# lucidrains/phenaki-pytorch

Measured on AMD Instinct MI355X. Metric: cvivit_encode_frames_per_sec, higher is better.
Workload: dtype bf16; 1 GPU; BASELINE configs[1]: C-ViViT (dim 512, patch 32, tpatch 2, depth 4+4, LFQ 65536) encode video -> token ids, (8,3,17,256,256) f32 per GPU resident in HBM; global_batch=8, parallelism=batch-shard x1, no data-path collective, hip_graph=True

## Files before the change

### phenaki_pytorch_amd/csrc/common.hpp

```cpp
#pragma once
#include <hip/hip_runtime.h>
#include <stdint.h>

namespace pk {

typedef float f32x4 __attribute__((ext_vector_type(4)));
typedef float f32x2 __attribute__((ext_vector_type(2)));
typedef __bf16 bf16x8_t __attribute__((ext_vector_type(8)));
typedef unsigned short u16;
typedef u16 u16x8 __attribute__((ext_vector_type(8)));
typedef u16 u16x4 __attribute__((ext_vector_type(4)));
typedef uint32_t u32x4 __attribute__((ext_vector_type(4)));
typedef uint32_t u32x2 __attribute__((ext_vector_type(2)));

struct bf16 { u16 v; };

struct bf16x3 { float v; };
struct bf16x3p { uint32_t v; };

typedef __bf16 bf16x2_native __attribute__((ext_vector_type(2)));
__device__ __forceinline__ u16 f2bf(float f) {
    return __builtin_bit_cast(u16, (__bf16)f);
}
__device__ __forceinline__ float bf2f(u16 h) {
// ... 104 lines not shown
}
__device__ __forceinline__ void store_elem(bf16x3p* p, float v) {
    const uintptr_t a = reinterpret_cast<uintptr_t>(p);
    char* blk = reinterpret_cast<char*>(a & ~(uintptr_t)127);
    const int o = (int)(a & 127) >> 1;
    const u16 h = f2bf(v);
    *reinterpret_cast<u16*>(blk + o) = h;
    *reinterpret_cast<u16*>(blk + 64 + o) = f2bf(v - bf2f(h));
}
__device__ __forceinline__ void store4(float* p, f32x4 v) { *reinterpret_cast<f32x4*>(p) = v; }
__device__ __forceinline__ void store4(bf16* p, f32x4 v) {
    *reinterpret_cast<u32x2*>(p) = u32x2{pack_bf2(v[0], v[1]), pack_bf2(v[2], v[3])};
}
__device__ __forceinline__ void store2(float* p, float a, float b) { *reinterpret_cast<f32x2*>(p) = f32x2{a, b}; }
__device__ __forceinline__ void store2(bf16* p, float a, float b) { *reinterpret_cast<uint32_t*>(p) = pack_bf2(a, b); }

__device__ __forceinline__ long xcd_contiguous_block(unsigned b, unsigned nblocks_padded) {
    return (long)(b & 7u) * (nblocks_padded >> 3) + (b >> 3);
}
__host__ __device__ inline unsigned xcd_padded_grid(long nblocks) { return (unsigned)(8 * ((nblocks + 7) / 8)); }

__device__ __forceinline__ float mul_rn(float a, float b) {
#pragma clang fp contract(off)
    return a * b;
}
__device__ __forceinline__ float add_rn(float a, float b) {
#pragma clang fp contract(off)
    return a + b;
}
__device__ __forceinline__ float wave_sum(float v) {
// ... 114 lines not shown
```

### phenaki_pytorch_amd/csrc/gemm.hip

```cpp
#include "gemm_dma.hpp"
#include "gemm_p8.hpp"

namespace pk {

enum { ACT_NONE = 0, ACT_GEGLU = 1, ACT_LEAKY = 2, ACT_RELU = 3 };

struct GemmEpilogue {
    const float* bias;
    const float* res;
    void* C;
    int ldr, ldc;
    int out_f32;
    int act;
    int vec_ok;
    void* C2;
    int ldc2;
    const float* ln_s; const float* ln_t; float ln_eps;
    const int* row_off; const int* col_off;
    float* stats_out; const float* ln_stats; int stats_np;
    int dup_rows;
};

constexpr int STATS_CHUNK = 32;

template <typename T, int TM, int TN, int WN>
__device__ __forceinline__ void gemm_epilogue_scalar(const f32x4 (&acc)[TM][TN], int M, int N, const GemmEpilogue& e, int m0, int n0) {
    const int lane = threadIdx.x & 63, wave = threadIdx.x >> 6;
    const int wm = wave / WN, wn = wave % WN, g = lane >> 4, lr = lane & 15;
    float* Cf = reinterpret_cast<float*>(e.C);
    T* Ct = reinterpret_cast<T*>(e.C);
#pragma unroll
    for (int i = 0; i < TM; ++i) {
        const int m = m0 + wm * 16 * TM + i * 16 + lr;
        if (m >= M) continue;
#pragma unroll
        for (int j = 0; j < TN; ++j) {
            const int n = n0 + wn * 16 * TN + j * 16 + g * 4;
            const f32x4 v = acc[i][j];
#pragma unroll
            for (int r = 0; r < 4; ++r) {
                const int nn = n + r;
                if (nn >= N) break;
                float x = v[r] + (e.bias ? e.bias[nn] : 0.f);
                if (e.act == ACT_GEGLU) {
                    if (r & 1) continue;
                    const float gate = (nn + 1 < N) ? v[r + 1] + (e.bias ? e.bias[nn + 1] : 0.f) : 0.f;
                    x = gelu_for<T>(gate) * x;
                    const size_t o = (size_t)m * e.ldc + (nn >> 1);
                    if (e.out_f32) Cf[o] = x; else store_elem(Ct + o, x);
                    continue;
                }
                if (e.act == ACT_LEAKY) x = x > 0.f ? x : 0.1f * x;
                if (e.act == ACT_RELU) x = fmaxf(x, 0.f);
                if (e.res) x += e.res[(size_t)m * e.ldr + nn];
                const size_t o = (size_t)m * e.ldc + nn;
                if (e.out_f32) Cf[o] = x; else store_elem(Ct + o, x);
            }
        }
    }
}

template <int TM> constexpr int epi_rows_per_round() { return TM > 2 ? 2 : TM; }

template <typename T, int TM, int TN, int WN = 2, bool LNF = false>
__device__ __forceinline__ void gemm_epilogue(const f32x4 (&acc)[TM][TN], int M, int N, const GemmEpilogue& e, int m0, int n0,
                                              const float* rsum = nullptr, const float* rsq = nullptr, int K = 1) {
    if (!e.vec_ok) {
        if (!LNF) gemm_epilogue_scalar<T, TM, TN, WN>(acc, M, N, e, m0, n0);
        return;
    }
    const int lane = threadIdx.x & 63, wave = threadIdx.x >> 6;
    const int wm = wave / WN, wn = wave % WN, g = lane >> 4, lr = lane & 15;
    float* __restrict__ Cf = reinterpret_cast<float*>(e.C);
    T* __restrict__ Ct = reinterpret_cast<T*>(e.C);
    const int mb = m0 + wm * 16 * TM + lr, nb = n0 + wn * 16 * TN + g * 4;
    f32x4 b4[TN], s4[TN], t4[TN];
    int coff[TN];
#pragma unroll
    for (int j = 0; j < TN; ++j) {
        const int nj = min(nb + j * 16, N - 4);
        b4[j] = e.bias ? *reinterpret_cast<const f32x4*>(e.bias + nj) : f32x4{0, 0, 0, 0};
        if (LNF) {
            s4[j] = *reinterpret_cast<const f32x4*>(e.ln_s + nj);
            t4[j] = *reinterpret_cast<const f32x4*>(e.ln_t + nj);
        }
        coff[j] = e.row_off ? e.col_off[nj] : nj;
    }
    constexpr int IB = epi_rows_per_round<TM>();
#pragma unroll
    for (int i0 = 0; i0 < TM; i0 += IB) {
        f32x4 r4[IB][TN];
        int roff[IB];
#pragma unroll
        for (int ii = 0; ii < IB; ++ii) {
            const int mi = min(mb + (i0 + ii) * 16, M - 1);
            roff[ii] = e.row_off ? e.row_off[mi] : 0;
            if (!LNF && e.res && e.act != ACT_GEGLU) {
#pragma unroll
                for (int j = 0; j < TN; ++j) r4[ii][j] = *reinterpret_cast<const f32x4*>(e.res + (size_t)mi * e.ldr + min(nb + j * 16, N - 4));
            } else {
#pragma unroll
                for (int j = 0; j < TN; ++j) r4[ii][j] = f32x4{0, 0, 0, 0};
            }
        }
#pragma unroll
        for (int ii = 0; ii < IB; ++ii) {
            const int i = i0 + ii, m = mb + i * 16;
            float mean = 0.f, rstd = 1.f;
            if (LNF) {
                const float inv_k = 1.0f / (float)K;
                mean = rsum[i] * inv_k;
                rstd = __builtin_amdgcn_rsqf(fmaxf(rsq[i] * inv_k - mean * mean, 0.f) + e.ln_eps);
            }
            float ps = 0.f, pq = 0.f;
#pragma unroll
            for (int j = 0; j < TN; ++j) {
                const int n = nb + j * 16;
                const bool live = m < M && n < N;
                f32x4 v = acc[i][j];
                if (LNF) {
#pragma unroll
                    for (int r = 0; r < 4; ++r) v[r] = rstd * (v[r] - mean * s4[j][r]) + t4[j][r];
                }
                v += b4[j];
                if (e.act == ACT_GEGLU) {
                    const float o0 = gelu_for<T>(v[1]) * v[0], o1 = gelu_for<T>(v[3]) * v[2];
                    const size_t o = (size_t)m * e.ldc + (n >> 1);
                    if (live) { if (e.out_f32) store2(Cf + o, o0, o1); else store2(Ct + o, o0, o1); }
                    continue;
                }
                if (e.act == ACT_LEAKY) {
#pragma unroll
                    for (int r = 0; r < 4; ++r) v[r] = v[r] > 0.f ? v[r] : 0.1f * v[r];
                }
                if (e.act == ACT_RELU) {
#pragma unroll
                    for (int r = 0; r < 4; ++r) v[r] = fmaxf(v[r], 0.f);
                }
                if (!LNF) v += r4[ii][j];
                else if (e.res && live) v += *reinterpret_cast<const f32x4*>(e.res + (size_t)m * e.ldr + n);
                if (live) {
                    const size_t o = e.row_off ? (size_t)((long)roff[ii] + (long)coff[j]) : (size_t)m * e.ldc + n;
                    if (e.out_f32) store4(Cf + o, v); else store4(Ct + o, v);
                    if (e.C2) store4(reinterpret_cast<bf16*>(e.C2) + (size_t)m * e.ldc2 + n, v);
                    if (e.dup_rows) {
                        const size_t od = o + (size_t)e.dup_rows * e.ldc;
                        if (e.out_f32) store4(Cf + od, v); else store4(Ct + od, v);
                        if (e.C2) store4(reinterpret_cast<bf16*>(e.C2) + (size_t)(m + e.dup_rows) * e.ldc2 + n, v);
                    }
                    if (TN == 2 && e.stats_out) {
#pragma unroll
                        for (int r = 0; r < 4; ++r) {
                            const float x = (sizeof(T) == 2 && (e.C2 || !e.out_f32)) ? bf2f(f2bf(v[r])) : v[r];
                            ps += x; pq += x * x;
                        }
                    }
                }
            }
            if (TN == 2 && e.stats_out) {
                ps += __shfl_xor(ps, 16); pq += __shfl_xor(pq, 16);
                ps += __shfl_xor(ps, 32); pq += __shfl_xor(pq, 32);
                const int chunk = (n0 + wn * 16 * TN) / STATS_CHUNK;
                if (g == 0 && m < M && chunk < e.stats_np)
                    reinterpret_cast<float2*>(e.stats_out)[(size_t)m * e.stats_np + chunk] = float2{ps, pq};
            }
        }
    }
}

template <typename T, typename TA, int TM, int TN>
__global__ __launch_bounds__(256) void gemm_kernel(const GemmOperands p, const GemmEpilogue e) {
    using Tile = GemmTile<T, TA, TM, TN>;
    extern __shared__ __attribute__((aligned(16))) char smem[];
    const int m0 = blockIdx.x * Tile::BM, n0 = blockIdx.y * Tile::BN;
    f32x4 acc[TM][TN];
#pragma unroll
    for (int i = 0; i < TM; ++i)
#pragma unroll
        for (int j = 0; j < TN; ++j) acc[i][j] = f32x4{0, 0, 0, 0};
    Tile::run(p, m0, n0, smem, acc);
    gemm_epilogue<T, TM, TN>(acc, p.M, p.N, e, m0, n0);
}

template <typename Tile>
constexpr int lds_waves_per_simd() {
    const int wgs = 163840 / Tile::SMEM, w = wgs * (Tile::THREADS / 64) / 4;
    return w < 1 ? 1 : (w > 8 ? 8 : w);
}

template <typename T, int TM, int TN, int WM, int WN, int STAGES, int ROWB, int PW, int LNF = 0>
__global__ __launch_bounds__(64 * (WM * WN + PW))
__attribute__((amdgpu_waves_per_eu(lds_waves_per_simd<GemmDma<T, TM, TN, WM, WN, STAGES, ROWB, PW>>(), 8)))
void gemm_dma_kernel(const GemmOperands p, const GemmEpilogue e, int a_nrows) {
    using Tile = GemmDma<T, TM, TN, WM, WN, STAGES, ROWB, PW>;
    extern __shared__ __attribute__((aligned(16))) char smem[];
    const int MT = (p.M + Tile::BM - 1) / Tile::BM, cmax = (MT + 7) / 8, NTn = (p.N + Tile::BN - 1) / Tile::BN;
    const int xcd = blockIdx.x & 7, idx = blockIdx.x >> 3;
    const int mstart = xcd * MT / 8, mcount = (xcd + 1) * MT / 8 - mstart;
    int m0, n0;
    if (p.plain_map) {
        if ((int)blockIdx.x >= MT * NTn) return;
        m0 = (blockIdx.x % MT) * Tile::BM;
        n0 = (blockIdx.x / MT) * Tile::BN;
    } else {
        int ml, ntile;
        if (!xcd_panel_tile(idx, cmax, mcount, NTn, p.panel, ml, ntile)) return;
        m0 = (mstart + ml) * Tile::BM;
        n0 = ntile * Tile::BN;
    }
    PK_TL_KERNEL(0);
    f32x4 acc[TM][TN];
#pragma unroll
    for (int i = 0; i < TM; ++i)
#pragma unroll
        for (int j = 0; j < TN; ++j) acc[i][j] = f32x4{0, 0, 0, 0};
    if constexpr (LNF == 1) {
        float rsum[TM], rsq[TM];
        if (!Tile::template run_stats<2>(p, a_nrows, m0, n0, smem, acc, rsum, rsq)) return;
        gemm_epilogue<T, TM, TN, WN, true>(acc, p.M, p.N, e, m0, n0, rsum, rsq, p.K);
    } else if constexpr (LNF == 2) {
        constexpr int TPR = Tile::THREADS / Tile::BM;
        static_assert(Tile::THREADS == TPR * Tile::BM && (TPR == 2 || TPR == 4), "2 or 4 threads per tile row");
        constexpr int NPRE = 16 / TPR;
        const int srow = threadIdx.x / TPR, sq4 = threadIdx.x % TPR;
        const int per = (e.stats_np + TPR - 1) / TPR, c0 = sq4 * per, c1 = min(c0 + per, e.stats_np);
        const float2* st = reinterpret_cast<const float2*>(e.ln_stats) + (size_t)min(m0 + srow, p.M - 1) * e.stats_np;
        float su = 0.f, sq = 0.f;
        for (int c = c0 + NPRE; c < c1; ++c) { const float2 pr = st[c]; su += pr.x; sq += pr.y; }
        float2 pre[NPRE];
#pragma unroll
        for (int u = 0; u < NPRE; ++u) pre[u] = c0 + u < c1 ? st[c0 + u] : float2{0.f, 0.f};
        if (!Tile::run(p, a_nrows, m0, n0, smem, acc)) return;
#pragma unroll
        for (int u = 0; u < NPRE; ++u) { su += pre[u].x; sq += pre[u].y; }
        su += __shfl_xor(su, 1); sq += __shfl_xor(sq, 1);
        if (TPR == 4) { su += __shfl_xor(su, 2); sq += __shfl_xor(sq, 2); }
        __syncthreads();
        float2* ls = reinterpret_cast<float2*>(smem);
        if (sq4 == 0) ls[srow] = float2{su, sq};
        __syncthreads();
        float rsum[TM], rsq[TM];
        const int lane = threadIdx.x & 63, wm = (threadIdx.x >> 6) / WN;
#pragma unroll
        for (int i = 0; i < TM; ++i) { const float2 pr = ls[wm * 16 * TM + i * 16 + (lane & 15)]; rsum[i] = pr.x; rsq[i] = pr.y; }
        gemm_epilogue<T, TM, TN, WN, true>(acc, p.M, p.N, e, m0, n0, rsum, rsq, p.K);
    } else {
        if (!Tile::run(p, a_nrows, m0, n0, smem, acc)) return;
        PK_TL_KERNEL(1);
        gemm_epilogue<T, TM, TN, WN>(acc, p.M, p.N, e, m0, n0);
        asm volatile("s_waitcnt vmcnt(0)" ::: "memory");
        PK_TL_KERNEL(2);
    }
}

template <typename T, int TM, int TN, int WM, int WN, int STAGES>
__global__ __launch_bounds__(64 * WM * WN)
__attribute__((amdgpu_waves_per_eu(lds_waves_per_simd<GemmDma<T, TM, TN, WM, WN, STAGES, 128, 0>>(), 8)))
void gemm_dma_splitk_kernel(GemmOperands p, GemmEpilogue e, int a_nrows, long batch_a, long batch_w, long batch_c) {
    using Tile = GemmDma<T, TM, TN, WM, WN, STAGES, 128, 0>;
    extern __shared__ __attribute__((aligned(16))) char smem[];
    const int z = blockIdx.y;
    p.A = reinterpret_cast<const char*>(p.A) + (size_t)z * batch_a;
    p.W = reinterpret_cast<const char*>(p.W) + (size_t)z * batch_w;
    e.C = reinterpret_cast<char*>(e.C) + (size_t)z * batch_c;
// ... 173 lines not shown
    const int eps_a = (dtype == 1 && !a_is_f32) ? 8 : 4;
    if (K % eps_w || ldw % eps_w || lda % eps_a) return PK_EALIGN;
    if (dtype == 1 && a_is_f32 && (K % 8)) return PK_EALIGN;
    if (!al16(A) || !al16(W)) return PK_EALIGN;
    if (dtype != 1 && !a_is_f32) return PK_EINVAL;
    if (dtype == 2 && C2) return PK_EINVAL;
    if (act == ACT_GEGLU && (N & 1)) return PK_EINVAL;
    if (a_rows && a_nrows <= 0) return PK_EINVAL;
    if (!a_rows) a_nrows = M;
    GemmOperands p{A, W, a_rows, lda, ldw, M, N, K, 0, N >= 8192 ? krot_default() : 0};
    GemmEpilogue e{bias, res, C, ldr, ldc, out_is_f32, act, 0, C2, ldc2, ln_s, ln_t, ln_eps, row_off, col_off, stats_out, ln_stats,
                   ((ln_stats ? K : N) + STATS_CHUNK - 1) / STATS_CHUNK, dup_rows};
    bool v = (N % 4 == 0) && (ldc % 4 == 0) && al16(C) && (!bias || al16(bias)) && (!res || (al16(res) && ldr % 4 == 0));
    if (act == ACT_GEGLU) v = v && (ldc % 2 == 0) && ((reinterpret_cast<uintptr_t>(C) & 7) == 0);
    e.vec_ok = v ? 1 : 0;
    if (C2 && (!v || !out_is_f32 || act == ACT_GEGLU || dtype != 1 || (ldc2 & 3) || (reinterpret_cast<uintptr_t>(C2) & 7))) return PK_EINVAL;
    if ((ln_s == nullptr) != (ln_t == nullptr)) return PK_EINVAL;
    if ((row_off == nullptr) != (col_off == nullptr)) return PK_EINVAL;
    if (row_off && (!v || !out_is_f32 || act == ACT_GEGLU || res || C2)) return PK_EINVAL;
    if (ln_stats && (!ln_s || stats_out || (reinterpret_cast<uintptr_t>(ln_stats) & 7))) return PK_EINVAL;
    if (stats_out && (!v || act == ACT_GEGLU || row_off || (reinterpret_cast<uintptr_t>(stats_out) & 7))) return PK_EINVAL;
    if (dup_rows < 0 || (dup_rows && (!v || act == ACT_GEGLU || row_off || stats_out || dup_rows < M))) return PK_EINVAL;
    hipStream_t s = reinterpret_cast<hipStream_t>(stream);

    const bool dma_ok = dma_possible(dtype, a_is_f32, N, K, lda, ldw, a_nrows);
    if (variant >= 100) { p.plain_map = 1; variant -= 100; }
    if (variant == 0) variant = auto_variant(dtype, a_is_f32, M, N, K, lda, ldw, a_nrows);
    if (variant >= 3 && !dma_ok) return PK_EINVAL;
    if (ln_s) {
        if (!dma_ok || !v || !al16(ln_s) || !al16(ln_t) || a_rows) return PK_EINVAL;
// ... 93 lines not shown
```

### phenaki_pytorch_amd/csrc/gemm_dma.hpp

```cpp
#pragma once
#include "gemm_core.hpp"

namespace pk {

__device__ __forceinline__ void dot2acc_bf16(float& d, uint32_t a, uint32_t b) {
    asm("v_dot2c_f32_bf16 %0, %1, %2" : "+v"(d) : "v"(a), "v"(b));
}
__device__ __forceinline__ void frag_stats(const Frag<bf16>& f, float& s, float& q, bool want_sq) {
    const uint32_t w0 = f.v[0], w1 = f.v[1], w2 = f.v[2], w3 = f.v[3];
    const uint32_t ones = 0x3f803f80u;
    dot2acc_bf16(s, w0, ones); dot2acc_bf16(s, w1, ones); dot2acc_bf16(s, w2, ones); dot2acc_bf16(s, w3, ones);
    if (want_sq) { dot2acc_bf16(q, w0, w0); dot2acc_bf16(q, w1, w1); dot2acc_bf16(q, w2, w2); dot2acc_bf16(q, w3, w3); }
}
__device__ __forceinline__ void frag_stats(const Frag<float>& f, float& s, float& q, bool want_sq) {
#pragma unroll
    for (int e = 0; e < 4; ++e) {
        s += f.lo[e] + f.hi[e];
        if (want_sq) q = fmaf(f.lo[e], f.lo[e], fmaf(f.hi[e], f.hi[e], q));
    }
}

#ifdef PK_TIMELINE
__device__ unsigned long long pk_tl[8 * 5 * 40];
#define PK_TL(slot) do { if (tl_on && kt < 38) pk_tl[(tl_wg * 40 + kt) * 5 + (slot)] = __builtin_amdgcn_s_memtime(); } while (0)
// ... 6 lines not shown
#define PK_TL_KERNEL(slot) do {} while (0)
#define PK_TL(slot) do {} while (0)
#endif

__device__ __forceinline__ void frag_stats(const Frag<bf16x3>& f, float& s, float& q, bool want_sq) {
    const uint32_t ones = 0x3f803f80u;
#pragma unroll
    for (int w = 0; w < 4; ++w) {
        dot2acc_bf16(s, f.hi[w], ones); dot2acc_bf16(s, f.lo[w], ones);
        if (want_sq) { dot2acc_bf16(q, f.hi[w], f.hi[w]); dot2acc_bf16(q, f.hi[w], f.lo[w]); dot2acc_bf16(q, f.hi[w], f.lo[w]); }
    }
}

template <int N> __device__ __forceinline__ void wait_vmcnt() { asm volatile("s_waitcnt vmcnt(%0)" ::"n"(N) : "memory"); }

template <typename T, int TM, int TN, int WM, int WN, int STAGES, int ROWB = 128, int PW = 0>
struct GemmDma {
    static_assert(ROWB == 128, "k-tile = 128 bytes per row (the 64-byte k-tile variants lost the round-1 sweep and were removed)");
    static constexpr int NW = WM * WN;
    static constexpr int BM = 16 * TM * WM, BN = 16 * TN * WN;
    static constexpr int RPI = 1024 / ROWB;
    static constexpr int SLOTS = ROWB / 16;
    static constexpr int NLW = PW > 0 ? PW : NW;
    static constexpr int THREADS = 64 * (NW + PW);
    static constexpr int IA = BM / (RPI * NLW), IW = BN / (RPI * NLW);
    static_assert(IA * RPI * NLW == BM && IW * RPI * NLW == BN, "tile rows must split evenly over the loading waves' DMA pieces");
    static constexpr int BK = ROWB / (int)sizeof(T);
    static constexpr int CH = BK / 32;
    static constexpr int STAGE_BYTES = (BM + BN) * ROWB;
    static constexpr int SMEM = STAGES * STAGE_BYTES;
    static constexpr int IPW = IA + IW;
// ... 38 lines not shown
        __amdgpu_buffer_rsrc_t rsW = __builtin_amdgcn_make_buffer_rsrc(const_cast<void*>(p.W), 0, bytesW, 0x00020000);

        const int lrow = lane / SLOTS, lslot = lane % SLOTS;
        const int srcslot = lslot ^ (lrow & 7);
        uint32_t offA[IA], offW[IW];
#pragma unroll
        for (int i = 0; i < IA; ++i) {
            const int row = (wave * IA + i) * RPI + lrow;
            int gm = m0 + row;
            const bool ok = gm < p.M;
            if (ok && p.a_rows) gm = p.a_rows[gm];
            offA[i] = ok ? (uint32_t)gm * (uint32_t)p.lda * SZ + srcslot * 16 : bytesA;
        }
#pragma unroll
        for (int i = 0; i < IW; ++i) {
            const int row = (wave * IW + i) * RPI + lrow;
            const int gn = n0 + row + ((p.w_gap_from > 0 && row >= p.w_gap_from) ? p.w_gap_rows : 0);
            offW[i] = gn < p.N ? (uint32_t)gn * (uint32_t)p.ldw * SZ + srcslot * 16 : bytesW;
        }

        const int nt = (p.K + BK - 1) / BK;
        const int rot = (p.krot && nt > 1) ? (int)(((blockIdx.x >> 3) + blockIdx.y) % (unsigned)nt) : 0;
        const int ktail_bytes = (p.K * SZ) % ROWB;
        const bool slot_in_tail = ktail_bytes == 0 || srcslot * 16 < ktail_bytes;
        auto issue = [&](int kt, int slot) {
            char* base = smem + slot * STAGE_BYTES;
            int kk = kt + rot;
            if (kk >= nt) kk -= nt;
            const int koff = kk * ROWB;
            const bool cut = kk == nt - 1 && !slot_in_tail;
#pragma unroll
// ... 68 lines not shown
```

### phenaki_pytorch_amd/csrc/qkv_attn.hip

```cpp
#include "gemm_dma.hpp"

namespace pk {

struct QkvAttnArgs {
    const void* xq; const void* xkv;
    const void* wq; const void* wkv;
    int ld, ldw;
    int S, n, h, K;
    int spt;
    const float* q_scale; const float* k_scale; float scale;
    const float* bias; long bias_hstride; int bias_ld;
    const float* slopes; int causal;
    void* O; int ldo;
    uint32_t recip;
    const float* q_ln_s;
};

template <typename T> using QaTile = GemmDma<T, 1, 4, 4, 1, 2, 128>;
template <typename T> using QaKvTile = GemmDma<T, 1, 8, 4, 1, 2, 128>;
constexpr int QA_SMEM = QaKvTile<bf16>::SMEM;
static_assert(QaKvTile<bf16x3>::SMEM == QA_SMEM, "the split-bf16 ring has the same bytes");

constexpr int QA_PLANE = 8192;
template <typename T> struct QaImg { static constexpr int PLANES = 1; };
template <> struct QaImg<bf16x3> { static constexpr int PLANES = 2; };
__device__ __forceinline__ void qa_put4(bf16, char* img, int off, f32x4 v) {
    *reinterpret_cast<u32x2*>(img + off) = u32x2{pack_bf2(v[0], v[1]), pack_bf2(v[2], v[3])};
}
__device__ __forceinline__ void qa_put4(bf16x3, char* img, int off, f32x4 v) {
    const uint32_t h0 = pack_bf2(v[0], v[1]), h1 = pack_bf2(v[2], v[3]);
// ... 4 lines not shown
}
__device__ __forceinline__ void qa_put1(bf16, char* img, int off, float v) { *reinterpret_cast<u16*>(img + off) = f2bf(v); }
__device__ __forceinline__ void qa_put1(bf16x3, char* img, int off, float v) {
    const u16 h = f2bf(v);
    *reinterpret_cast<u16*>(img + off) = h;
    *reinterpret_cast<u16*>(img + QA_PLANE + off) = f2bf(v - bf2f(h));
}
__device__ __forceinline__ void qa_get(Frag<bf16>& f, const char* img, int off) { f.v = *reinterpret_cast<const u32x4*>(img + off); }
__device__ __forceinline__ void qa_get(Frag<bf16x3>& f, const char* img, int off) {
    f.hi = *reinterpret_cast<const u32x4*>(img + off);
    f.lo = *reinterpret_cast<const u32x4*>(img + QA_PLANE + off);
}

__device__ __forceinline__ int qa_kperm(int f, int i) { return (f >> 1) * 32 + (i >> 2) * 8 + (f & 1) * 4 + (i & 3); }
__device__ __forceinline__ int qa_ksw(int row) { return ((row >> 1) & 1) | (((row >> 3) & 3) << 1); }

template <typename T>
__device__ __forceinline__ void qa_project_q(const GemmOperands& p, int M, int m0, int hh, int K, const float* q_scale, float scale,
                                             const float* q_ln_s, char* smem, char* Qs) {
    const int lane = threadIdx.x & 63, g = lane >> 4, lr = lane & 15;
    const int rq = __builtin_amdgcn_readfirstlane(threadIdx.x >> 6) * 16 + lr;
    f32x4 acc[1][4];
#pragma unroll
    for (int j = 0; j < 4; ++j) acc[0][j] = f32x4{0, 0, 0, 0};
    if (q_ln_s) {
        float rsum[1], rsq[1];
        (void)QaTile<T>::template run_stats<1>(p, M, m0, hh * 64, smem, acc, rsum, rsq);
        const float mean = rsum[0] / (float)K;
#pragma unroll
        for (int j = 0; j < 4; ++j) {
// ... 73 lines not shown
        ss += __shfl_xor(ss, 32, 64);
        const float inv = 1.0f / fmaxf(sqrtf(ss), 1e-12f);
#pragma unroll
        for (int j = 0; j < 4; ++j) {
            const f32x4 sc = *reinterpret_cast<const f32x4*>(a.k_scale + j * 16 + g * 4);
            f32x4 v = acc[0][j];
#pragma unroll
            for (int r = 0; r < 4; ++r) v[r] *= inv * sc[r];
            const int slot = (2 * j + (g >> 1)) ^ qa_ksw(rq);
            qa_put4(T{}, Ks, rq * 128 + (slot << 4) + (g & 1) * 8, v);
        }
#pragma unroll
        for (int j = 0; j < 4; ++j)
#pragma unroll
            for (int r = 0; r < 4; ++r) {
                const int d = j * 16 + g * 4 + r;
                qa_put1(T{}, Vts, d * 128 + ((((rq >> 3) ^ (d & 7))) << 4) + (rq & 7) * 2, acc[0][4 + j][r]);
            }
    }
    asm volatile("s_waitcnt lgkmcnt(0)" ::: "memory");
    __builtin_amdgcn_s_barrier();

    f32x4 st[4];
#pragma unroll
    for (int f = 0; f < 4; ++f) st[f] = f32x4{0, 0, 0, 0};
#pragma unroll
    for (int f = 0; f < 4; ++f) {
        const int krow = qa_kperm(f, lr);
#pragma unroll
        for (int c = 0; c < 2; ++c) {
            Frag<T> fk;
            qa_get(fk, Ks, krow * 128 + (((c * 4 + g) ^ qa_ksw(krow)) << 4));
// ... 42 lines not shown
    for (int e = 0; e < 16; ++e) { pr[e] = __expf(pr[e] - mx); ls += pr[e]; }
    ls += __shfl_xor(ls, 16, 64);
    ls += __shfl_xor(ls, 32, 64);
    f32x4 o[4];
#pragma unroll
    for (int df = 0; df < 4; ++df) o[df] = f32x4{0, 0, 0, 0};
#pragma unroll
    for (int kc = 0; kc < 2; ++kc) {
        Frag<T> fp;
        {
            const float p8[8] = {pr[kc * 8 + 0], pr[kc * 8 + 1], pr[kc * 8 + 2], pr[kc * 8 + 3], pr[kc * 8 + 4], pr[kc * 8 + 5], pr[kc * 8 + 6], pr[kc * 8 + 7]};
            frag_from_f32(fp, p8);
        }
#pragma unroll
        for (int df = 0; df < 4; ++df) {
            const int d = df * 16 + lr;
            Frag<T> fv;
            qa_get(fv, Vts, d * 128 + (((kc * 4 + g) ^ (d & 7)) << 4));
            o[df] = mma(fv, fp, o[df]);
        }
    }
    if (!qvalid) return;
    const float inv = 1.0f / ls;
    T* orow = reinterpret_cast<T*>(a.O) + (size_t)(m0 + rq) * a.ldo + hh * 64;
#pragma unroll
    for (int df = 0; df < 4; ++df) store4(orow + df * 16 + g * 4, o[df] * inv);
}

struct QAttnCachedArgs {
    const void* xq; const void* wq; int ld, ldw;
    int S, n, h, K;
    const float* q_scale; float scale; const float* q_ln_s;
    const void* Kp; const void* Vt; int nk_pad, nk, nnull;
    const unsigned char* kmask; int n_kv;
    void* O; int ldo;
};

template <typename T, bool NK64>
__global__ __launch_bounds__(256) void q_attn_cached_kernel(const QAttnCachedArgs a) {
    extern __shared__ __attribute__((aligned(16))) char smem[];
    constexpr int NPL = QaImg<T>::PLANES;
    char* Qs = smem + QaTile<T>::SMEM;
    char* Ks = Qs + NPL * QA_PLANE;
    char* Vts = smem;
    const int M = a.S * a.n;
    const int tiles = M / 64;
    const int xcd = blockIdx.x & 7, idx = blockIdx.x >> 3;
    const int tile = (idx / a.h) * 8 + xcd, hh = idx % a.h;
    if (tile >= tiles) return;
    const int m0 = tile * 64;
// ... 2 lines not shown
    const int wave = __builtin_amdgcn_readfirstlane(threadIdx.x >> 6);
    const int rq = wave * 16 + lr;

    GemmOperands p;
    p.a_rows = nullptr;
    p.lda = a.ld; p.ldw = a.ldw;
    p.M = M; p.K = a.K;
    p.plain_map = 0; p.krot = 0;
    p.w_gap_from = 0; p.w_gap_rows = 0;
    p.A = a.xq; p.W = a.wq; p.N = a.h * 64;
    qa_project_q<T>(p, M, m0, hh, a.K, a.q_scale, a.scale, a.q_ln_s, smem, Qs);

    {
        const size_t sh = (size_t)s * a.h + hh;
        const int row = threadIdx.x >> 2, part = threadIdx.x & 3;
        const u32x4 zero = u32x4{0, 0, 0, 0};
        if constexpr (NPL == 1) {
            const bf16* krow = reinterpret_cast<const bf16*>(a.Kp) + (sh * a.nk_pad + row) * 64;
            const bf16* vrow = reinterpret_cast<const bf16*>(a.Vt) + (sh * 64 + row) * a.nk_pad;
#pragma unroll
            for (int q = 0; q < 2; ++q) {
                const int slot = part * 2 + q;
                const u32x4 kv = row < a.nk_pad ? *reinterpret_cast<const u32x4*>(krow + slot * 8) : zero;
                *reinterpret_cast<u32x4*>(Ks + row * 128 + ((slot ^ qa_ksw(row)) << 4)) = kv;
                const u32x4 vv = slot * 8 < a.nk_pad ? *reinterpret_cast<const u32x4*>(vrow + slot * 8) : zero;
                *reinterpret_cast<u32x4*>(Vts + row * 128 + ((slot ^ (row & 7)) << 4)) = vv;
            }
        } else {
            const char* krow = reinterpret_cast<const char*>(a.Kp) + (sh * a.nk_pad + row) * 256;
            const char* vrow = reinterpret_cast<const char*>(a.Vt) + (sh * 64 + row) * (size_t)a.nk_pad * 4;
            u32x4 kv[4], vv[4];
#pragma unroll
            for (int q = 0; q < 4; ++q) {
                const int sp = part * 4 + q;
                kv[q] = row < a.nk_pad ? *reinterpret_cast<const u32x4*>(krow + sp * 16) : zero;
                vv[q] = (sp >> 3) * 32 < a.nk_pad ? *reinterpret_cast<const u32x4*>(vrow + sp * 16) : zero;
            }
#pragma unroll
            for (int q = 0; q < 4; ++q) {
                const int sp = part * 4 + q;
                const int plane = (sp >> 2) & 1, slot = (sp >> 3) * 4 + (sp & 3);
                *reinterpret_cast<u32x4*>(Ks + plane * QA_PLANE + row * 128 + ((slot ^ qa_ksw(row)) << 4)) = kv[q];
                *reinterpret_cast<u32x4*>(Vts + plane * QA_PLANE + row * 128 + ((slot ^ (row & 7)) << 4)) = vv[q];
            }
        }
    }
    asm volatile("s_waitcnt lgkmcnt(0)" ::: "memory");
    __builtin_amdgcn_s_barrier();

    constexpr int NF = NK64 ? 4 : 2;
    Frag<T> fq[2];
#pragma unroll
    for (int c = 0; c < 2; ++c) qa_get(fq[c], Qs, rq * 128 + (((c * 4 + g) ^ (rq & 7)) << 4));
    f32x4 st[NF];
#pragma unroll
    for (int f = 0; f < NF; ++f) {
        st[f] = f32x4{0, 0, 0, 0};
        const int krow = qa_kperm(f, lr);
// ... 25 lines not shown
    for (int e = 0; e < 4 * NF; ++e) { pr[e] = __expf(pr[e] - mx); ls += pr[e]; }
    ls += __shfl_xor(ls, 16, 64);
    ls += __shfl_xor(ls, 32, 64);
    f32x4 o[4];
#pragma unroll
    for (int df = 0; df < 4; ++df) o[df] = f32x4{0, 0, 0, 0};
#pragma unroll
    for (int kc = 0; kc < NF / 2; ++kc) {
        Frag<T> fp;
        {
            const float p8[8] = {pr[kc * 8 + 0], pr[kc * 8 + 1], pr[kc * 8 + 2], pr[kc * 8 + 3], pr[kc * 8 + 4], pr[kc * 8 + 5], pr[kc * 8 + 6], pr[kc * 8 + 7]};
            frag_from_f32(fp, p8);
        }
#pragma unroll
        for (int df = 0; df < 4; ++df) {
            const int d = df * 16 + lr;
            Frag<T> fv;
            qa_get(fv, Vts, d * 128 + (((kc * 4 + g) ^ (d & 7)) << 4));
            o[df] = mma(fv, fp, o[df]);
        }
    }
    const float inv = 1.0f / ls;
    T* orow = reinterpret_cast<T*>(a.O) + (size_t)(m0 + rq) * a.ldo + hh * 64;
#pragma unroll
    for (int df = 0; df < 4; ++df) store4(orow + df * 16 + g * 4, o[df] * inv);
}

}
using namespace pk;

extern "C" int pk_qkv_attn(int dtype, const void* xq, const void* xkv, int ld, const void* wq, const void* wkv, int ldw, int S, int n, int h,
                           int K, const float* q_scale, const float* k_scale, float scale, const float* bias, long bias_hstride,
                           int bias_ld, const float* slopes, int causal, void* O, int ldo, const float* q_ln_s, void* stream) {
    if (dtype != 1 && dtype != 2) return PK_EINVAL;
    if (!xq || !xkv || !wq || !wkv || !q_scale || !k_scale || !O || S <= 0 || n <= 0 || n > 64 || h <= 0 || K <= 0) return PK_EINVAL;
    auto mis = [](const void* ptr) { return (reinterpret_cast<uintptr_t>(ptr) & 15) != 0; };
    const int q = dtype == 1 ? 7 : 3, bk = dtype == 1 ? 64 : 32, esz = dtype == 1 ? 2 : 4;
    if ((K & q) || (ld & q) || (ldw & q) || (ldo & 3) || mis(xq) || mis(xkv) || mis(wq) || mis(wkv) || mis(q_scale) || mis(k_scale) ||
        (reinterpret_cast<uintptr_t>(O) & (dtype == 1 ? 7 : 15)) || (bias && mis(bias))) return PK_EALIGN;
    if (ldw < (K + bk - 1) / bk * bk) return PK_EINVAL;
    const long M = (long)S * n;
    if ((size_t)M * ld * esz >= 0xFFFFFFF0ull || (size_t)2 * h * 64 * ldw * esz >= 0xFFFFFFF0ull) return PK_EINVAL;
    QkvAttnArgs a;
    a.xq = xq; a.xkv = xkv; a.wq = wq; a.wkv = wkv; a.ld = ld; a.ldw = ldw;
    a.S = S; a.n = n; a.h = h; a.K = K; a.spt = 64 / n;
    a.q_scale = q_scale; a.k_scale = k_scale; a.scale = scale;
    a.bias = bias; a.bias_hstride = bias_hstride; a.bias_ld = bias_ld;
    a.slopes = slopes; a.causal = causal;
    a.O = O; a.ldo = ldo;
    a.recip = (65536u + (uint32_t)n - 1u) / (uint32_t)n;
    a.q_ln_s = q_ln_s;
    if (q_ln_s && mis(q_ln_s)) return PK_EALIGN;
    const int tiles = (S + a.spt - 1) / a.spt;
    dim3 grid(8 * ((tiles + 7) / 8) * h);
    hipStream_t st = reinterpret_cast<hipStream_t>(stream);
    if (dtype == 1) hipLaunchKernelGGL(qkv_attn_kernel<bf16>, grid, dim3(256), QA_SMEM, st, a);
    else hipLaunchKernelGGL(qkv_attn_kernel<bf16x3>, grid, dim3(256), QA_SMEM, st, a);
    PK_CHECK_LAUNCH();
    return PK_OK;
}

extern "C" int pk_q_attn_cached(int dtype, const void* xq, int ld, const void* wq, int ldw, int S, int n, int h, int K, const float* q_scale,
                                float scale, const float* q_ln_s, const void* Kp, const void* Vt, int nk_pad, int n_kv, int nnull,
                                const unsigned char* kmask, void* O, int ldo, void* stream) {
    if (dtype != 1 && dtype != 2) return PK_EINVAL;
    if (!xq || !wq || !q_scale || !Kp || !Vt || !O || S <= 0 || n <= 0 || (n & 63) || h <= 0 || K <= 0 || n_kv <= 0 || nnull < 0) return PK_EINVAL;
    const int nk = nnull + n_kv;
    if (nk > 64 || nk_pad < nk || nk_pad > 64 || (nk_pad & 31)) return PK_EINVAL;
    auto mis = [](const void* ptr) { return (reinterpret_cast<uintptr_t>(ptr) & 15) != 0; };
    const int q = dtype == 1 ? 7 : 3, bk = dtype == 1 ? 64 : 32, esz = dtype == 1 ? 2 : 4;
    if ((K & q) || (ld & q) || (ldw & q) || (ldo & 3) || mis(xq) || mis(wq) || mis(q_scale) || mis(Kp) || mis(Vt) ||
        (reinterpret_cast<uintptr_t>(O) & (dtype == 1 ? 7 : 15)) || (q_ln_s && mis(q_ln_s))) return PK_EALIGN;
    if (dtype == 2 && ((reinterpret_cast<uintptr_t>(Kp) | reinterpret_cast<uintptr_t>(Vt)) & 127)) return PK_EALIGN;
    if (ldw < (K + bk - 1) / bk * bk) return PK_EINVAL;
    const long M = (long)S * n;
    if ((size_t)M * ld * esz >= 0xFFFFFFF0ull || (size_t)h * 64 * ldw * esz >= 0xFFFFFFF0ull) return PK_EINVAL;
    QAttnCachedArgs a{xq, wq, ld, ldw, S, n, h, K, q_scale, scale, q_ln_s, Kp, Vt, nk_pad, nk, nnull, kmask, n_kv, O, ldo};
    const int tiles = (int)(M / 64);
    dim3 grid(8 * ((tiles + 7) / 8) * h);
    hipStream_t st = reinterpret_cast<hipStream_t>(stream);
    if (dtype == 1) {
        constexpr int lds = QaTile<bf16>::SMEM + 2 * QA_PLANE;
        if (nk_pad > 32) hipLaunchKernelGGL((q_attn_cached_kernel<bf16, true>), grid, dim3(256), lds, st, a);
        else hipLaunchKernelGGL((q_attn_cached_kernel<bf16, false>), grid, dim3(256), lds, st, a);
    } else {
        constexpr int lds = QaTile<bf16x3>::SMEM + 4 * QA_PLANE;
        if (nk_pad > 32) hipLaunchKernelGGL((q_attn_cached_kernel<bf16x3, true>), grid, dim3(256), lds, st, a);
        else hipLaunchKernelGGL((q_attn_cached_kernel<bf16x3, false>), grid, dim3(256), lds, st, a);
    }
    PK_CHECK_LAUNCH();
    return PK_OK;
}
// ... 1 lines not shown
```

Before: 179,700 frames/s.

## Permute weight rows and V layout so epilogues write adjacent columns in wide stores

For TN=2 GEMM tiles, W rows are remapped at load time so each lane group's accumulator fragments cover adjacent output columns. The epilogue can then issue 16-byte stores (store8) in place of scattered 8-byte ones, and the GEGLU path writes four outputs per lane at once. The attention kernels apply the same idea by permuting V-transpose rows in LDS, with a new swizzle, so each lane writes 16 contiguous head-dim outputs. The aim is fewer, wider global stores. In exchange, the row-statistics reduction gets more complex and adds extra shuffles, and a fallback path is needed when alignment checks fail.

```diff
diff --git a/phenaki_pytorch_amd/csrc/common.hpp b/phenaki_pytorch_amd/csrc/common.hpp
--- a/phenaki_pytorch_amd/csrc/common.hpp
+++ b/phenaki_pytorch_amd/csrc/common.hpp
@@ -142,6 +142,11 @@
 }
 __device__ __forceinline__ void store2(float* p, float a, float b) { *reinterpret_cast<f32x2*>(p) = f32x2{a, b}; }
 __device__ __forceinline__ void store2(bf16* p, float a, float b) { *reinterpret_cast<uint32_t*>(p) = pack_bf2(a, b); }
+__device__ __forceinline__ void store8(bf16* p, f32x4 a, f32x4 b) {
+    *reinterpret_cast<u32x4*>(p) = u32x4{pack_bf2(a[0], a[1]), pack_bf2(a[2], a[3]), pack_bf2(b[0], b[1]), pack_bf2(b[2], b[3])};
+}
+__device__ __forceinline__ void store8(float* p, f32x4 a, f32x4 b) { store4(p, a); store4(p + 4, b); }
+__device__ __forceinline__ void store8(bf16x3* p, f32x4 a, f32x4 b) { store4(p, a); store4(p + 4, b); }
 
 __device__ __forceinline__ long xcd_contiguous_block(unsigned b, unsigned nblocks_padded) {
     return (long)(b & 7u) * (nblocks_padded >> 3) + (b >> 3);
diff --git a/phenaki_pytorch_amd/csrc/gemm.hip b/phenaki_pytorch_amd/csrc/gemm.hip
--- a/phenaki_pytorch_amd/csrc/gemm.hip
+++ b/phenaki_pytorch_amd/csrc/gemm.hip
@@ -19,11 +19,12 @@
     const int* row_off; const int* col_off;
     float* stats_out; const float* ln_stats; int stats_np;
     int dup_rows;
+    int wide_ok;
 };
 
 constexpr int STATS_CHUNK = 32;
 
-template <typename T, int TM, int TN, int WN>
+template <typename T, int TM, int TN, int WN, bool ADJ = false>
 __device__ __forceinline__ void gemm_epilogue_scalar(const f32x4 (&acc)[TM][TN], int M, int N, const GemmEpilogue& e, int m0, int n0) {
     const int lane = threadIdx.x & 63, wave = threadIdx.x >> 6;
     const int wm = wave / WN, wn = wave % WN, g = lane >> 4, lr = lane & 15;
@@ -35,7 +36,7 @@
         if (m >= M) continue;
 #pragma unroll
         for (int j = 0; j < TN; ++j) {
-            const int n = n0 + wn * 16 * TN + j * 16 + g * 4;
+            const int n = n0 + wn * 16 * TN + (ADJ ? g * 4 * TN + j * 4 : j * 16 + g * 4);
             const f32x4 v = acc[i][j];
 #pragma unroll
             for (int r = 0; r < 4; ++r) {
@@ -62,23 +63,25 @@
 
 template <int TM> constexpr int epi_rows_per_round() { return TM > 2 ? 2 : TM; }
 
-template <typename T, int TM, int TN, int WN = 2, bool LNF = false>
+template <typename T, int TM, int TN, int WN = 2, bool LNF = false, bool ADJ = false>
 __device__ __forceinline__ void gemm_epilogue(const f32x4 (&acc)[TM][TN], int M, int N, const GemmEpilogue& e, int m0, int n0,
                                               const float* rsum = nullptr, const float* rsq = nullptr, int K = 1) {
+    static_assert(!ADJ || TN == 2, "the adjacent-column map is built for the TN = 2 tiles");
     if (!e.vec_ok) {
-        if (!LNF) gemm_epilogue_scalar<T, TM, TN, WN>(acc, M, N, e, m0, n0);
+        if (!LNF) gemm_epilogue_scalar<T, TM, TN, WN, ADJ>(acc, M, N, e, m0, n0);
         return;
     }
     const int lane = threadIdx.x & 63, wave = threadIdx.x >> 6;
     const int wm = wave / WN, wn = wave % WN, g = lane >> 4, lr = lane & 15;
     float* __restrict__ Cf = reinterpret_cast<float*>(e.C);
     T* __restrict__ Ct = reinterpret_cast<T*>(e.C);
-    const int mb = m0 + wm * 16 * TM + lr, nb = n0 + wn * 16 * TN + g * 4;
+    constexpr int JS = ADJ ? 4 : 16;
+    const int mb = m0 + wm * 16 * TM + lr, nb = n0 + wn * 16 * TN + g * (ADJ ? 4 * TN : 4);
     f32x4 b4[TN], s4[TN], t4[TN];
     int coff[TN];
 #pragma unroll
     for (int j = 0; j < TN; ++j) {
-        const int nj = min(nb + j * 16, N - 4);
+        const int nj = min(nb + j * JS, N - 4);
         b4[j] = e.bias ? *reinterpret_cast<const f32x4*>(e.bias + nj) : f32x4{0, 0, 0, 0};
         if (LNF) {
             s4[j] = *reinterpret_cast<const f32x4*>(e.ln_s + nj);
@@ -97,7 +100,7 @@
             roff[ii] = e.row_off ? e.row_off[mi] : 0;
             if (!LNF && e.res && e.act != ACT_GEGLU) {
 #pragma unroll
-                for (int j = 0; j < TN; ++j) r4[ii][j] = *reinterpret_cast<const f32x4*>(e.res + (size_t)mi * e.ldr + min(nb + j * 16, N - 4));
+                for (int j = 0; j < TN; ++j) r4[ii][j] = *reinterpret_cast<const f32x4*>(e.res + (size_t)mi * e.ldr + min(nb + j * JS, N - 4));
             } else {
 #pragma unroll
                 for (int j = 0; j < TN; ++j) r4[ii][j] = f32x4{0, 0, 0, 0};
@@ -112,10 +115,11 @@
                 mean = rsum[i] * inv_k;
                 rstd = __builtin_amdgcn_rsqf(fmaxf(rsq[i] * inv_k - mean * mean, 0.f) + e.ln_eps);
             }
-            float ps = 0.f, pq = 0.f;
+            const bool both = ADJ && m < M && nb + 4 * TN <= N;
+            f32x4 vv[TN];
 #pragma unroll
             for (int j = 0; j < TN; ++j) {
-                const int n = nb + j * 16;
+                const int n = nb + j * JS;
                 const bool live = m < M && n < N;
                 f32x4 v = acc[i][j];
                 if (LNF) {
@@ -124,9 +128,7 @@
                 }
                 v += b4[j];
                 if (e.act == ACT_GEGLU) {
-                    const float o0 = gelu_for<T>(v[1]) * v[0], o1 = gelu_for<T>(v[3]) * v[2];
-                    const size_t o = (size_t)m * e.ldc + (n >> 1);
-                    if (live) { if (e.out_f32) store2(Cf + o, o0, o1); else store2(Ct + o, o0, o1); }
+                    vv[j] = f32x4{gelu_for<T>(v[1]) * v[0], gelu_for<T>(v[3]) * v[2], 0.f, 0.f};
                     continue;
                 }
                 if (e.act == ACT_LEAKY) {
@@ -139,7 +141,38 @@
                 }
                 if (!LNF) v += r4[ii][j];
                 else if (e.res && live) v += *reinterpret_cast<const f32x4*>(e.res + (size_t)m * e.ldr + n);
-                if (live) {
+                vv[j] = v;
+            }
+            if (e.act == ACT_GEGLU) {
+                if (both) {
+                    const f32x4 o4 = {vv[0][0], vv[0][1], vv[TN - 1][0], vv[TN - 1][1]};
+                    const size_t o = (size_t)m * e.ldc + (nb >> 1);
+                    if (e.out_f32) store4(Cf + o, o4); else store4(Ct + o, o4);
+                } else {
+#pragma unroll
+                    for (int j = 0; j < TN; ++j) {
+                        const int n = nb + j * JS;
+                        const size_t o = (size_t)m * e.ldc + (n >> 1);
+                        if (m < M && n < N) { if (e.out_f32) store2(Cf + o, vv[j][0], vv[j][1]); else store2(Ct + o, vv[j][0], vv[j][1]); }
+                    }
+                }
+                continue;
+            }
+            if (both && e.wide_ok) {
+                const size_t o = (size_t)m * e.ldc + nb;
+                if (e.out_f32) store8(Cf + o, vv[0], vv[TN - 1]); else store8(Ct + o, vv[0], vv[TN - 1]);
+                if (e.C2) store8(reinterpret_cast<bf16*>(e.C2) + (size_t)m * e.ldc2 + nb, vv[0], vv[TN - 1]);
+                if (e.dup_rows) {
+                    const size_t od = o + (size_t)e.dup_rows * e.ldc;
+                    if (e.out_f32) store8(Cf + od, vv[0], vv[TN - 1]); else store8(Ct + od, vv[0], vv[TN - 1]);
+                    if (e.C2) store8(reinterpret_cast<bf16*>(e.C2) + (size_t)(m + e.dup_rows) * e.ldc2 + nb, vv[0], vv[TN - 1]);
+                }
+            } else {
+#pragma unroll
+                for (int j = 0; j < TN; ++j) {
+                    const int n = nb + j * JS;
+                    if (!(m < M && n < N)) continue;
+                    const f32x4 v = vv[j];
                     const size_t o = e.row_off ? (size_t)((long)roff[ii] + (long)coff[j]) : (size_t)m * e.ldc + n;
                     if (e.out_f32) store4(Cf + o, v); else store4(Ct + o, v);
                     if (e.C2) store4(reinterpret_cast<bf16*>(e.C2) + (size_t)m * e.ldc2 + n, v);
@@ -148,20 +181,40 @@
                         if (e.out_f32) store4(Cf + od, v); else store4(Ct + od, v);
                         if (e.C2) store4(reinterpret_cast<bf16*>(e.C2) + (size_t)(m + e.dup_rows) * e.ldc2 + n, v);
                     }
-                    if (TN == 2 && e.stats_out) {
-#pragma unroll
-                        for (int r = 0; r < 4; ++r) {
-                            const float x = (sizeof(T) == 2 && (e.C2 || !e.out_f32)) ? bf2f(f2bf(v[r])) : v[r];
-                            ps += x; pq += x * x;
+                }
+            }
+            if (TN == 2 && e.stats_out) {
+                const auto seen = [&](float x) { return (sizeof(T) == 2 && (e.C2 || !e.out_f32)) ? bf2f(f2bf(x)) : x; };
+                const int chunk = (n0 + wn * 16 * TN) / STATS_CHUNK;
+                float ps = 0.f, pq = 0.f;
+                if (!ADJ) {
+#pragma unroll
+                    for (int j = 0; j < TN; ++j) {
+                        if (!(m < M && nb + j * JS < N)) continue;
+#pragma unroll
+                        for (int r = 0; r < 4; ++r) { const float x = seen(vv[j][r]); ps += x; pq += x * x; }
+                    }
+                    ps += __shfl_xor(ps, 16); pq += __shfl_xor(pq, 16);
+                    ps += __shfl_xor(ps, 32); pq += __shfl_xor(pq, 32);
+                } else {
+                    float sa[TN], qa[TN];
+#pragma unroll
+                    for (int j = 0; j < TN; ++j) {
+                        sa[j] = 0.f; qa[j] = 0.f;
+                        const bool live = m < M && nb + j * JS < N;
+#pragma unroll
+                        for (int r = 0; r < 4; ++r) { const float x = seen(vv[j][r]); if (live) { sa[j] += x; qa[j] += x * x; } }
+                        const float so = __shfl_xor(sa[j], 32), qo = __shfl_xor(qa[j], 32);
+                        if (g >= 2) {
+                            sa[j] = so; qa[j] = qo;
+#pragma unroll
+                            for (int r = 0; r < 4; ++r) { const float x = seen(vv[j][r]); if (live) { sa[j] += x; qa[j] += x * x; } }
                         }
                     }
-                }
-            }
-            if (TN == 2 && e.stats_out) {
-                ps += __shfl_xor(ps, 16); pq += __shfl_xor(pq, 16);
-                ps += __shfl_xor(ps, 32); pq += __shfl_xor(pq, 32);
-                const int chunk = (n0 + wn * 16 * TN) / STATS_CHUNK;
-                if (g == 0 && m < M && chunk < e.stats_np)
+                    ps = sa[0] + sa[TN - 1]; pq = qa[0] + qa[TN - 1];
+                    ps += __shfl_xor(ps, 16); pq += __shfl_xor(pq, 16);
+                }
+                if (g == (ADJ ? 2 : 0) && m < M && chunk < e.stats_np)
                     reinterpret_cast<float2*>(e.stats_out)[(size_t)m * e.stats_np + chunk] = float2{ps, pq};
             }
         }
@@ -192,7 +245,8 @@
 __global__ __launch_bounds__(64 * (WM * WN + PW))
 __attribute__((amdgpu_waves_per_eu(lds_waves_per_simd<GemmDma<T, TM, TN, WM, WN, STAGES, ROWB, PW>>(), 8)))
 void gemm_dma_kernel(const GemmOperands p, const GemmEpilogue e, int a_nrows) {
-    using Tile = GemmDma<T, TM, TN, WM, WN, STAGES, ROWB, PW>;
+    constexpr bool ADJ = TN == 2;
+    using Tile = GemmDma<T, TM, TN, WM, WN, STAGES, ROWB, PW, ADJ>;
     extern __shared__ __attribute__((aligned(16))) char smem[];
     const int MT = (p.M + Tile::BM - 1) / Tile::BM, cmax = (MT + 7) / 8, NTn = (p.N + Tile::BN - 1) / Tile::BN;
     const int xcd = blockIdx.x & 7, idx = blockIdx.x >> 3;
@@ -217,7 +271,7 @@
     if constexpr (LNF == 1) {
         float rsum[TM], rsq[TM];
         if (!Tile::template run_stats<2>(p, a_nrows, m0, n0, smem, acc, rsum, rsq)) return;
-        gemm_epilogue<T, TM, TN, WN, true>(acc, p.M, p.N, e, m0, n0, rsum, rsq, p.K);
+        gemm_epilogue<T, TM, TN, WN, true, ADJ>(acc, p.M, p.N, e, m0, n0, rsum, rsq, p.K);
     } else if constexpr (LNF == 2) {
         constexpr int TPR = Tile::THREADS / Tile::BM;
         static_assert(Tile::THREADS == TPR * Tile::BM && (TPR == 2 || TPR == 4), "2 or 4 threads per tile row");
@@ -243,11 +297,11 @@
         const int lane = threadIdx.x & 63, wm = (threadIdx.x >> 6) / WN;
 #pragma unroll
         for (int i = 0; i < TM; ++i) { const float2 pr = ls[wm * 16 * TM + i * 16 + (lane & 15)]; rsum[i] = pr.x; rsq[i] = pr.y; }
-        gemm_epilogue<T, TM, TN, WN, true>(acc, p.M, p.N, e, m0, n0, rsum, rsq, p.K);
+        gemm_epilogue<T, TM, TN, WN, true, ADJ>(acc, p.M, p.N, e, m0, n0, rsum, rsq, p.K);
     } else {
         if (!Tile::run(p, a_nrows, m0, n0, smem, acc)) return;
         PK_TL_KERNEL(1);
-        gemm_epilogue<T, TM, TN, WN>(acc, p.M, p.N, e, m0, n0);
+        gemm_epilogue<T, TM, TN, WN, false, ADJ>(acc, p.M, p.N, e, m0, n0);
         asm volatile("s_waitcnt vmcnt(0)" ::: "memory");
         PK_TL_KERNEL(2);
     }
@@ -451,6 +505,7 @@
     bool v = (N % 4 == 0) && (ldc % 4 == 0) && al16(C) && (!bias || al16(bias)) && (!res || (al16(res) && ldr % 4 == 0));
     if (act == ACT_GEGLU) v = v && (ldc % 2 == 0) && ((reinterpret_cast<uintptr_t>(C) & 7) == 0);
     e.vec_ok = v ? 1 : 0;
+    e.wide_ok = (v && !row_off && (dtype != 1 || out_is_f32 || ldc % 8 == 0) && (!C2 || (ldc2 % 8 == 0 && al16(C2)))) ? 1 : 0;
     if (C2 && (!v || !out_is_f32 || act == ACT_GEGLU || dtype != 1 || (ldc2 & 3) || (reinterpret_cast<uintptr_t>(C2) & 7))) return PK_EINVAL;
     if ((ln_s == nullptr) != (ln_t == nullptr)) return PK_EINVAL;
     if ((row_off == nullptr) != (col_off == nullptr)) return PK_EINVAL;
diff --git a/phenaki_pytorch_amd/csrc/gemm_dma.hpp b/phenaki_pytorch_amd/csrc/gemm_dma.hpp
--- a/phenaki_pytorch_amd/csrc/gemm_dma.hpp
+++ b/phenaki_pytorch_amd/csrc/gemm_dma.hpp
@@ -44,7 +44,7 @@
 
 template <int N> __device__ __forceinline__ void wait_vmcnt() { asm volatile("s_waitcnt vmcnt(%0)" ::"n"(N) : "memory"); }
 
-template <typename T, int TM, int TN, int WM, int WN, int STAGES, int ROWB = 128, int PW = 0>
+template <typename T, int TM, int TN, int WM, int WN, int STAGES, int ROWB = 128, int PW = 0, bool ADJ = false>
 struct GemmDma {
     static_assert(ROWB == 128, "k-tile = 128 bytes per row (the 64-byte k-tile variants lost the round-1 sweep and were removed)");
     static constexpr int NW = WM * WN;
@@ -113,7 +113,8 @@
         }
 #pragma unroll
         for (int i = 0; i < IW; ++i) {
-            const int row = (wave * IW + i) * RPI + lrow;
+            int row = (wave * IW + i) * RPI + lrow;
+            if (ADJ) row = row / (16 * TN) * (16 * TN) + ((row & 15) >> 2) * (4 * TN) + (row / 16 % TN) * 4 + (row & 3);
             const int gn = n0 + row + ((p.w_gap_from > 0 && row >= p.w_gap_from) ? p.w_gap_rows : 0);
             offW[i] = gn < p.N ? (uint32_t)gn * (uint32_t)p.ldw * SZ + srcslot * 16 : bytesW;
         }
diff --git a/phenaki_pytorch_amd/csrc/qkv_attn.hip b/phenaki_pytorch_amd/csrc/qkv_attn.hip
--- a/phenaki_pytorch_amd/csrc/qkv_attn.hip
+++ b/phenaki_pytorch_amd/csrc/qkv_attn.hip
@@ -14,6 +14,7 @@
     void* O; int ldo;
     uint32_t recip;
     const float* q_ln_s;
+    int o_wide;
 };
 
 template <typename T> using QaTile = GemmDma<T, 1, 4, 4, 1, 2, 128>;
@@ -48,6 +49,18 @@
 
 __device__ __forceinline__ int qa_kperm(int f, int i) { return (f >> 1) * 32 + (i >> 2) * 8 + (f & 1) * 4 + (i & 3); }
 __device__ __forceinline__ int qa_ksw(int row) { return ((row >> 1) & 1) | (((row >> 3) & 3) << 1); }
+__device__ __forceinline__ int qa_vrow(int d) { return ((d >> 2) & 3) * 16 + (d >> 4) * 4 + (d & 3); }
+__device__ __forceinline__ int qa_vsw(int row) { return (row ^ (row >> 4)) & 7; }
+template <typename T>
+__device__ __forceinline__ void qa_store_o(T* orow, const f32x4 (&o)[4], float inv, bool wide) {
+    if (wide) {
+        store8(orow, o[0] * inv, o[1] * inv);
+        store8(orow + 8, o[2] * inv, o[3] * inv);
+    } else {
+#pragma unroll
+        for (int df = 0; df < 4; ++df) store4(orow + df * 4, o[df] * inv);
+    }
+}
 
 template <typename T>
 __device__ __forceinline__ void qa_project_q(const GemmOperands& p, int M, int m0, int hh, int K, const float* q_scale, float scale,
@@ -151,8 +164,8 @@
         for (int j = 0; j < 4; ++j)
 #pragma unroll
             for (int r = 0; r < 4; ++r) {
-                const int d = j * 16 + g * 4 + r;
-                qa_put1(T{}, Vts, d * 128 + ((((rq >> 3) ^ (d & 7))) << 4) + (rq & 7) * 2, acc[0][4 + j][r]);
+                const int vr = qa_vrow(j * 16 + g * 4 + r);
+                qa_put1(T{}, Vts, vr * 128 + ((((rq >> 3) ^ qa_vsw(vr))) << 4) + (rq & 7) * 2, acc[0][4 + j][r]);
             }
     }
     asm volatile("s_waitcnt lgkmcnt(0)" ::: "memory");
@@ -225,17 +238,16 @@
         }
 #pragma unroll
         for (int df = 0; df < 4; ++df) {
-            const int d = df * 16 + lr;
+            const int vr = df * 16 + lr;
             Frag<T> fv;
-            qa_get(fv, Vts, d * 128 + (((kc * 4 + g) ^ (d & 7)) << 4));
+            qa_get(fv, Vts, vr * 128 + (((kc * 4 + g) ^ qa_vsw(vr)) << 4));
             o[df] = mma(fv, fp, o[df]);
         }
     }
     if (!qvalid) return;
     const float inv = 1.0f / ls;
-    T* orow = reinterpret_cast<T*>(a.O) + (size_t)(m0 + rq) * a.ldo + hh * 64;
-#pragma unroll
-    for (int df = 0; df < 4; ++df) store4(orow + df * 16 + g * 4, o[df] * inv);
+    T* orow = reinterpret_cast<T*>(a.O) + (size_t)(m0 + rq) * a.ldo + hh * 64 + g * 16;
+    qa_store_o(orow, o, inv, a.o_wide != 0);
 }
 
 struct QAttnCachedArgs {
@@ -245,6 +257,7 @@
     const void* Kp; const void* Vt; int nk_pad, nk, nnull;
     const unsigned char* kmask; int n_kv;
     void* O; int ldo;
+    int o_wide;
 };
 
 template <typename T, bool NK64>
@@ -277,6 +290,7 @@
     {
         const size_t sh = (size_t)s * a.h + hh;
         const int row = threadIdx.x >> 2, part = threadIdx.x & 3;
+        const int vr = qa_vrow(row);
         const u32x4 zero = u32x4{0, 0, 0, 0};
         if constexpr (NPL == 1) {
             const bf16* krow = reinterpret_cast<const bf16*>(a.Kp) + (sh * a.nk_pad + row) * 64;
@@ -287,7 +301,7 @@
                 const u32x4 kv = row < a.nk_pad ? *reinterpret_cast<const u32x4*>(krow + slot * 8) : zero;
                 *reinterpret_cast<u32x4*>(Ks + row * 128 + ((slot ^ qa_ksw(row)) << 4)) = kv;
                 const u32x4 vv = slot * 8 < a.nk_pad ? *reinterpret_cast<const u32x4*>(vrow + slot * 8) : zero;
-                *reinterpret_cast<u32x4*>(Vts + row * 128 + ((slot ^ (row & 7)) << 4)) = vv;
+                *reinterpret_cast<u32x4*>(Vts + vr * 128 + ((slot ^ qa_vsw(vr)) << 4)) = vv;
             }
         } else {
             const char* krow = reinterpret_cast<const char*>(a.Kp) + (sh * a.nk_pad + row) * 256;
@@ -304,7 +318,7 @@
                 const int sp = part * 4 + q;
                 const int plane = (sp >> 2) & 1, slot = (sp >> 3) * 4 + (sp & 3);
                 *reinterpret_cast<u32x4*>(Ks + plane * QA_PLANE + row * 128 + ((slot ^ qa_ksw(row)) << 4)) = kv[q];
-                *reinterpret_cast<u32x4*>(Vts + plane * QA_PLANE + row * 128 + ((slot ^ (row & 7)) << 4)) = vv[q];
+                *reinterpret_cast<u32x4*>(Vts + plane * QA_PLANE + vr * 128 + ((slot ^ qa_vsw(vr)) << 4)) = vv[q];
             }
         }
     }
@@ -360,16 +374,15 @@
         }
 #pragma unroll
         for (int df = 0; df < 4; ++df) {
-            const int d = df * 16 + lr;
+            const int vr = df * 16 + lr;
             Frag<T> fv;
-            qa_get(fv, Vts, d * 128 + (((kc * 4 + g) ^ (d & 7)) << 4));
+            qa_get(fv, Vts, vr * 128 + (((kc * 4 + g) ^ qa_vsw(vr)) << 4));
             o[df] = mma(fv, fp, o[df]);
         }
     }
     const float inv = 1.0f / ls;
-    T* orow = reinterpret_cast<T*>(a.O) + (size_t)(m0 + rq) * a.ldo + hh * 64;
-#pragma unroll
-    for (int df = 0; df < 4; ++df) store4(orow + df * 16 + g * 4, o[df] * inv);
+    T* orow = reinterpret_cast<T*>(a.O) + (size_t)(m0 + rq) * a.ldo + hh * 64 + g * 16;
+    qa_store_o(orow, o, inv, a.o_wide != 0);
 }
 
 }
@@ -396,6 +409,7 @@
     a.O = O; a.ldo = ldo;
     a.recip = (65536u + (uint32_t)n - 1u) / (uint32_t)n;
     a.q_ln_s = q_ln_s;
+    a.o_wide = (dtype != 1 || (!mis(O) && (ldo & 7) == 0)) ? 1 : 0;
     if (q_ln_s && mis(q_ln_s)) return PK_EALIGN;
     const int tiles = (S + a.spt - 1) / a.spt;
     dim3 grid(8 * ((tiles + 7) / 8) * h);
@@ -421,7 +435,8 @@
     if (ldw < (K + bk - 1) / bk * bk) return PK_EINVAL;
     const long M = (long)S * n;
     if ((size_t)M * ld * esz >= 0xFFFFFFF0ull || (size_t)h * 64 * ldw * esz >= 0xFFFFFFF0ull) return PK_EINVAL;
-    QAttnCachedArgs a{xq, wq, ld, ldw, S, n, h, K, q_scale, scale, q_ln_s, Kp, Vt, nk_pad, nk, nnull, kmask, n_kv, O, ldo};
+    QAttnCachedArgs a{xq, wq, ld, ldw, S, n, h, K, q_scale, scale, q_ln_s, Kp, Vt, nk_pad, nk, nnull, kmask, n_kv, O, ldo,
+                      (dtype != 1 || (!mis(O) && (ldo & 7) == 0)) ? 1 : 0};
     const int tiles = (int)(M / 64);
     dim3 grid(8 * ((tiles + 7) / 8) * h);
     hipStream_t st = reinterpret_cast<hipStream_t>(stream);
```

New measurement: 178,600 frames/s. No clear change (-0.6%).
